# 4ment/physher

Hardware: NVIDIA B200
Metric: lnL+gradient throughput (site patterns x tree nodes per second) (higher is better)
Workload: dtype f64

## Files before the change

### physher_b200/csrc/phb_nuc4.cu

```cuda
#include "phb_ctx.cuh"

#include <math.h>
#include <stdlib.h>
#include <string.h>

#define NUC4_CHUNK PHBC_WALK_CHUNK
#define NUC4_NT 256
#ifndef NUC4_L2PF
#define NUC4_L2PF 1
#endif

struct Nuc4Params {
	int T, N, C, P, PB, root;
	int n_post, n_pre, nslots, ntiles;
	int include_root_freqs, compat;
	int nbatch, phases;
	long long mats_stride;
	int post_first_tips, pre_first_tips;
	double threshold;
	const uint8_t *tip_codes;
	const double *weights;
	const double *props;
	const phbc_post_op *post_ops;
	const phbc_pre_op *pre_ops;
	const double *post_mats;
	const double *pre_mats;
	double *lower;
	double *gacc;
	double *gstat;
	double *cta_lnl;
	double *pattern_lnl;
	double freqs[4];
	double fq[4];
	double wroot[4];
	double FQ[16];
	double FQ2[16];
	const double *rates;
	double *hacc;
};

__device__ __forceinline__ void matvec_smem(const double *__restrict__ M, const double (&x)[4], double (&y)[4]) {
	const double2 *M2 = reinterpret_cast<const double2 *>(M);
#pragma unroll
	for (int i = 0; i < 4; i++) {
		const double2 a = M2[2 * i], b = M2[2 * i + 1];
		y[i] = fma(a.x, x[0], fma(a.y, x[1], fma(b.x, x[2], b.y * x[3])));
	}
}

__device__ __forceinline__ void tip_message(const double *__restrict__ M, unsigned code, double (&y)[4]) {
	if (__all_sync(0xffffffffu, code < 4u)) {
#pragma unroll
		for (int i = 0; i < 4; i++) y[i] = M[4 * i + code];
	} else {
		double x[4];
#pragma unroll
		for (int j = 0; j < 4; j++) x[j] = (code < 4u ? code == (unsigned)j : ((code >> j) & 1u)) ? 1.0 : 0.0;
		matvec_smem(M, x, y);
		if (code == 4u) y[0] = y[1] = y[2] = y[3] = 1.0;
	}
}

#define NUC4_SLOT_BYTES (2 * NUC4_NT * 16)
#define NUC4_ROW_BYTES (NUC4_NT * 32)

__device__ __forceinline__ void cell_load(const unsigned char *cell, double (&x)[4]) {
	const double2 lo = *reinterpret_cast<const double2 *>(cell);
	const double2 hi = *reinterpret_cast<const double2 *>(cell + NUC4_NT * 16);
	x[0] = lo.x, x[1] = lo.y, x[2] = hi.x, x[3] = hi.y;
}
__device__ __forceinline__ void cell_store(unsigned char *cell, const double (&x)[4]) {
	*reinterpret_cast<double2 *>(cell) = make_double2(x[0], x[1]);
	*reinterpret_cast<double2 *>(cell + NUC4_NT * 16) = make_double2(x[2], x[3]);
}
__device__ __forceinline__ void row_load(const unsigned char *cell, double (&x)[4]) {
	const double2 lo = __ldcs(reinterpret_cast<const double2 *>(cell));
	const double2 hi = __ldcs(reinterpret_cast<const double2 *>(cell + NUC4_NT * 16));
	x[0] = lo.x, x[1] = lo.y, x[2] = hi.x, x[3] = hi.y;
}
__device__ __forceinline__ void row_store(unsigned char *cell, const double (&x)[4]) {
	__stcs(reinterpret_cast<double2 *>(cell), make_double2(x[0], x[1]));
	__stcs(reinterpret_cast<double2 *>(cell + NUC4_NT * 16), make_double2(x[2], x[3]));
}

struct Nuc4Stage {
	uint32_t desc_off, mat_off, code_off, bytes;
};
__host__ __device__ constexpr Nuc4Stage nuc4_stage_layout(int C, int PB) {
	return Nuc4Stage{64u, (uint32_t)(64 + NUC4_CHUNK * 48), (uint32_t)(64 + NUC4_CHUNK * 48 + NUC4_CHUNK * 3 * C * 128),
	                 (uint32_t)((64 + NUC4_CHUNK * 48 + NUC4_CHUNK * 3 * C * 128 + 2 * NUC4_CHUNK * PB + 127) & ~127)};
}

__device__ __forceinline__ double butterfly4(double v0, double v1, double v2, double v3, int lane) {
	const bool h16 = lane & 16, h8 = lane & 8;
	const double r01 = (h16 ? v1 : v0) + __shfl_xor_sync(0xffffffffu, h16 ? v0 : v1, 16);
	const double r23 = (h16 ? v3 : v2) + __shfl_xor_sync(0xffffffffu, h16 ? v2 : v3, 16);
	double r = (h8 ? r23 : r01) + __shfl_xor_sync(0xffffffffu, h8 ? r01 : r23, 8);
	r += __shfl_xor_sync(0xffffffffu, r, 4);
	r += __shfl_xor_sync(0xffffffffu, r, 2);
	r += __shfl_xor_sync(0xffffffffu, r, 1);
	return r;
}
__device__ __forceinline__ double butterfly2(double v0, double v1, int lane) {
	const bool h16 = lane & 16;
	double r = (h16 ? v1 : v0) + __shfl_xor_sync(0xffffffffu, h16 ? v0 : v1, 16);
	r += __shfl_xor_sync(0xffffffffu, r, 8);
	r += __shfl_xor_sync(0xffffffffu, r, 4);
	r += __shfl_xor_sync(0xffffffffu, r, 2);
	r += __shfl_xor_sync(0xffffffffu, r, 1);
	return r;
}

__device__ __forceinline__ void tip_vector(unsigned code, double (&x)[4]) {
#pragma unroll
	for (int j = 0; j < 4; j++) x[j] = (code < 4u ? code == (unsigned)j : (code == 4u || ((code >> j) & 1u))) ? 1.0 : 0.0;
}

template <int PPT>
__device__ __forceinline__ void gstat_add(const double (&t)[PPT][4], const double (&x)[PPT][4], double *row, int lane) {
	double v[16];
#pragma unroll
	for (int i = 0; i < 4; i++)
#pragma unroll
		for (int j = 0; j < 4; j++) {
			double a = t[0][i] * x[0][j];
#pragma unroll
			for (int u = 1; u < PPT; u++) a = fma(t[u][i], x[u][j], a);
			v[4 * i + j] = a;
		}
#pragma unroll
	for (int w = 8, off = 16; w >= 1; w >>= 1, off >>= 1) {
		const bool h = lane & off;
#pragma unroll
		for (int k = 0; k < w; k++) {
			const double keep = h ? v[w + k] : v[k], send = h ? v[k] : v[w + k];
			v[k] = keep + __shfl_xor_sync(0xffffffffu, send, off);
		}
	}
	v[0] += __shfl_xor_sync(0xffffffffu, v[0], 1);
	if (!(lane & 1)) red_add_f64(row + (lane >> 1), v[0]);
}

template <int PPT>
__device__ __forceinline__ void matvec_smem_n(const double *__restrict__ M, const double (&x)[PPT][4], double (&y)[PPT][4]) {
	const double2 *M2 = reinterpret_cast<const double2 *>(M);
#pragma unroll
	for (int i = 0; i < 4; i++) {
		const double2 a = M2[2 * i], b = M2[2 * i + 1];
#pragma unroll
		for (int u = 0; u < PPT; u++) y[u][i] = fma(a.x, x[u][0], fma(a.y, x[u][1], fma(b.x, x[u][2], b.y * x[u][3])));
	}
}

template <int C, bool SCALE, int GRAD, int PPT>
__global__ void __launch_bounds__(NUC4_NT / PPT, GRAD == 3 ? (PPT == 1 ? 1 : 2) : 3) k_nuc4_walk(const Nuc4Params prm) {
	extern __shared__ __align__(128) unsigned char smem_raw[];
	constexpr int PB = NUC4_NT / C;
	constexpr int NTHR = NUC4_NT / PPT;
	constexpr int PBT = PB / PPT;
	static_assert(PBT % 32 == 0 || PPT == 1, "a warp must not mix categories");
	static_assert(GRAD != 3 || !SCALE, "the Hessian walk is unscaled (rescaled evaluations take the resident-partials route)");
	constexpr bool RECOMP = GRAD == 1 && !SCALE;
	const int tid = threadIdx.x, lane = tid & 31, warp = tid >> 5;
	const int c = tid / PBT, pl0 = tid - c * PBT;
	const int cell0 = c * PB + pl0;
	constexpr Nuc4Stage lay = nuc4_stage_layout(C, PB);
	uint64_t *bars = reinterpret_cast<uint64_t *>(smem_raw);
	unsigned char *stage0 = smem_raw;
	unsigned char *slot_cell = stage0 + 2 * lay.bytes + cell0 * 16;
	double *xch = reinterpret_cast<double *>(stage0 + 2 * lay.bytes + (size_t)prm.nslots * NUC4_SLOT_BYTES);
	double *invLw = xch + (SCALE ? (GRAD == 2 ? 5 : 4) : (GRAD == 3 ? 2 : 1)) * C * PB;
	double *sfslot = invLw + PB;
	const uint32_t my_mat = lay.mat_off + c * 128;
	const uint32_t my_code = lay.code_off + pl0;

	if (tid == 0) {
		mbar_init(&bars[0], 1);
		mbar_init(&bars[1], 1);
		asm volatile("fence.mbarrier_init.release.cluster;" ::: "memory");
	}
	__syncthreads();

	uint32_t loads = 0;
	const double prop_c = (C == 1) ? 1.0 : prm.props[c];
	double cta_lnl = 0.0;
	unsigned char *row_cell = GRAD ? reinterpret_cast<unsigned char *>(prm.lower) + (size_t)blockIdx.x * prm.n_post * NUC4_ROW_BYTES + cell0 * 16 : nullptr;
	double *my_gacc = nullptr;
	double *my_gstat = GRAD == 2 ? prm.gstat + ((size_t)blockIdx.x * (NTHR / 32) + warp) * prm.N * 16 : nullptr;
	double *my_hacc = GRAD == 3 ? prm.hacc + ((size_t)blockIdx.x * (NTHR / 32) + warp) * prm.N : nullptr;
	const double rate_c = GRAD == 3 ? prm.rates[c] : 0.0;

	constexpr int PF_LPR = PPT * 2 * 4;
	const int pf_row = (lane / PF_LPR) & 1, pf_q = lane % PF_LPR;
	const bool pf_on = GRAD && lane < 2 * PF_LPR;
	const unsigned char *pf_base = GRAD ? row_cell - lane * 16 + ((pf_q >> 3) * PBT) * 16 + ((pf_q >> 2) & 1) * (NUC4_NT * 16) + (pf_q & 3) * 128 : nullptr;

	const long long nitems = (long long)prm.ntiles * prm.nbatch;
	const bool strided = prm.nbatch == 1;
	const int item0 = strided ? (int)blockIdx.x : (int)(blockIdx.x * nitems / gridDim.x);
	const int item1 = strided ? (int)nitems : (int)((blockIdx.x + 1) * nitems / gridDim.x);
	const int item_step = strided ? (int)gridDim.x : 1;
	const int b_first = strided ? 0 : item0 / prm.ntiles;
	int cur_b = -1;
	auto flush_lnl = [&](int b) {
		if (lane == 0) prm.cta_lnl[((size_t)blockIdx.x * prm.phases + (b - b_first)) * (NTHR / 32) + warp] = (c == 0) ? cta_lnl : 0.0;
	};

	for (int item = item0; item < item1; item += item_step) {
		const int bsmp = item / prm.ntiles, tile = item - bsmp * prm.ntiles;
		if (bsmp != cur_b) {
			if (cur_b >= 0) flush_lnl(cur_b);
			cur_b = bsmp;
			cta_lnl = 0.0;
			if (GRAD) my_gacc = prm.gacc + (((size_t)blockIdx.x * prm.phases + (bsmp - b_first)) * (NTHR / 32) + warp) * prm.N;
		}
		const uint8_t *tile_codes_post = prm.tip_codes + (size_t)tile * prm.T * PB;
		const uint8_t *tile_codes_pre = prm.tip_codes + ((size_t)prm.ntiles + tile) * prm.T * PB;

		double out[PPT][4];
		double sf_acc[PPT];
#pragma unroll
		for (int u = 0; u < PPT; u++) out[u][0] = out[u][1] = out[u][2] = out[u][3] = 1.0, sf_acc[u] = 0.0;
		{
			const int nchunks = (prm.n_post + NUC4_CHUNK - 1) / NUC4_CHUNK;
			auto issue = [&](int ch, uint32_t ld, int tips) {
				const int first = ch * NUC4_CHUNK;
				const int cnt = min(NUC4_CHUNK, prm.n_post - first);
				unsigned char *dst = stage0 + (ld & 1) * lay.bytes;
				const uint32_t dbytes = cnt * (uint32_t)sizeof(phbc_post_op), mbytes = cnt * 3 * C * 128;
				const uint32_t cbytes = (tips & 31) * PB;
				mbar_expect_tx(&bars[ld & 1], dbytes + mbytes + cbytes);
				bulk_g2s(dst + lay.desc_off, prm.post_ops + first, dbytes, &bars[ld & 1]);
				bulk_g2s(dst + lay.mat_off, prm.post_mats + (size_t)cur_b * prm.mats_stride + (size_t)first * 3 * C * 16, mbytes, &bars[ld & 1]);
				if (cbytes) bulk_g2s(dst + lay.code_off, tile_codes_post + (size_t)(tips >> 5) * PB, cbytes, &bars[ld & 1]);
			};
			if (tid == 0) issue(0, loads, prm.post_first_tips);
			for (int ch = 0; ch < nchunks; ch++) {
				mbar_wait(&bars[loads & 1], (loads >> 1) & 1);
				const unsigned char *st = stage0 + (loads & 1) * lay.bytes;
				const phbc_post_op *desc = reinterpret_cast<const phbc_post_op *>(st + lay.desc_off);
				if (tid == 0 && ch + 1 < nchunks) issue(ch + 1, loads + 1, desc[0].next_tips);
				const unsigned char *mats = st + my_mat;
				const uint8_t *cds = st + my_code;
				const int first = ch * NUC4_CHUNK;
				const int cnt = min(NUC4_CHUNK, prm.n_post - first);
#pragma unroll 1
				for (int j = 0; j < cnt; j++) {
					const int kind = (desc[j].a_kind & 0xff) + desc[j].b_kind;
					const bool keep_row = !(RECOMP && (desc[j].a_kind & PHBC_POST_NO_ROW));
					const int a_idx = desc[j].a_idx, b_idx = desc[j].b_idx, dst_slot = desc[j].dst_slot;
					const double *MN = reinterpret_cast<const double *>(mats + (j * 3 + 0) * C * 128);
					const double *MA = reinterpret_cast<const double *>(mats + (j * 3 + 1) * C * 128);
					const double *MB = reinterpret_cast<const double *>(mats + (j * 3 + 2) * C * 128);
					double ma[PPT][4], lw[PPT][4];
					double sf_in[PPT];
#pragma unroll
					for (int u = 0; u < PPT; u++) sf_in[u] = 0.0;
					if (kind == 0) {
#pragma unroll
						for (int u = 0; u < PPT; u++) {
							tip_message(MA, cds[a_idx * PB + u * PBT], ma[u]);
							tip_message(MB, cds[b_idx * PB + u * PBT], out[u]);
						}
					} else {
						if (SCALE) {
#pragma unroll
							for (int u = 0; u < PPT; u++) sf_in[u] = sf_acc[u];
						}
						if (kind == 1) {
#pragma unroll
							for (int u = 0; u < PPT; u++) tip_message(MA, cds[a_idx * PB + u * PBT], ma[u]);
						} else {
#pragma unroll
							for (int u = 0; u < PPT; u++) {
								cell_load(slot_cell + a_idx * NUC4_SLOT_BYTES + u * PBT * 16, ma[u]);
								if (SCALE) sf_in[u] += sfslot[a_idx * NUC4_NT + cell0 + u * PBT];
							}
						}
					}
#pragma unroll
					for (int u = 0; u < PPT; u++)
#pragma unroll
						for (int i = 0; i < 4; i++) lw[u][i] = ma[u][i] * out[u][i];
					if (SCALE) {
						double *mx = xch + ((first + j) & 1) * C * PB;
#pragma unroll
						for (int u = 0; u < PPT; u++) mx[cell0 + u * PBT] = fmax(fmax(lw[u][0], lw[u][1]), fmax(lw[u][2], lw[u][3]));
						__syncthreads();
#pragma unroll
						for (int u = 0; u < PPT; u++) {
							const int pl = pl0 + u * PBT;
							double m = mx[pl];
							for (int cc = 1; cc < C; cc++) m = fmax(m, mx[cc * PB + pl]);
							double sf = 0.0;
							if (m < prm.threshold) {
#pragma unroll
								for (int i = 0; i < 4; i++) lw[u][i] /= m;
								sf = log(m);
							}
							sf_acc[u] = sf + sf_in[u];
							if (dst_slot >= 0) sfslot[dst_slot * NUC4_NT + cell0 + u * PBT] = sf_acc[u];
						}
					}
					matvec_smem_n<PPT>(MN, lw, out);
#pragma unroll
					for (int u = 0; u < PPT; u++) {
						if (dst_slot >= 0) cell_store(slot_cell + dst_slot * NUC4_SLOT_BYTES + u * PBT * 16, out[u]);
						if (GRAD && keep_row) row_store(row_cell + (size_t)(unsigned)(first + j) * NUC4_ROW_BYTES + u * PBT * 16, out[u]);
					}
				}
				loads++;
				__syncthreads();
			}
		}

		{
#pragma unroll
			for (int u = 0; u < PPT; u++) {
				double site = prm.freqs[0] * out[u][0] + prm.freqs[1] * out[u][1] + prm.freqs[2] * out[u][2] + prm.freqs[3] * out[u][3];
				xch[cell0 + u * PBT] = site * prop_c;
			}
			__syncthreads();
			if (c == 0) {
				double v = 0.0;
#pragma unroll
				for (int u = 0; u < PPT; u++) {
					const int pl = pl0 + u * PBT;
					const int p = tile * PB + pl;
					const bool live = p < prm.P;
					double L = xch[pl];
					for (int cc = 1; cc < C; cc++) L += xch[cc * PB + pl];
					double plk = log(L);
					if (SCALE) plk += sf_acc[u];
					const double w = live ? prm.weights[p] : 0.0;
					if (live && prm.nbatch == 1) prm.pattern_lnl[p] = plk;
					invLw[pl] = w / L;
					if (GRAD == 3) invLw[PB + pl] = 1.0 / L;
					v += live ? plk * w : 0.0;
				}
				v = phb_warp_sum(v);
				if (lane == 0) cta_lnl += v;
			}
			__syncthreads();
		}

		if (GRAD) {
			double sgrad[PPT], wk[PPT], rinv[PPT];
#pragma unroll
			for (int u = 0; u < PPT; u++) {
				const int pl = pl0 + u * PBT;
				const int p = tile * PB + pl;
				sgrad[u] = invLw[pl];
				wk[u] = p < prm.P ? prm.weights[p] : 0.0;
				rinv[u] = GRAD == 3 ? invLw[PB + pl] : 0.0;
			}
			if (GRAD == 2) {
				double r[4];
#pragma unroll
				for (int i = 0; i < 4; i++) {
					r[i] = sgrad[0] * out[0][i];
#pragma unroll
					for (int u = 1; u < PPT; u++) r[i] = fma(sgrad[u], out[u][i], r[i]);
				}
				const double tot = butterfly4(r[0], r[1], r[2], r[3], lane);
				if ((lane & 7) == 0) red_add_f64(my_gstat + (size_t)prm.root * 16 + (((lane >> 4) & 1) | ((lane >> 2) & 2)), tot);
			}
			const int nchunks = (prm.n_pre + NUC4_CHUNK - 1) / NUC4_CHUNK;
			auto issue = [&](int ch, uint32_t ld, int tips) {
				const int first = ch * NUC4_CHUNK;
				const int cnt = min(NUC4_CHUNK, prm.n_pre - first);
				unsigned char *dst = stage0 + (ld & 1) * lay.bytes;
				const uint32_t dbytes = cnt * (uint32_t)sizeof(phbc_pre_op), mbytes = cnt * 3 * C * 128;
				const uint32_t cbytes = (tips & 31) * PB;
				mbar_expect_tx(&bars[ld & 1], dbytes + mbytes + cbytes);
				bulk_g2s(dst + lay.desc_off, prm.pre_ops + first, dbytes, &bars[ld & 1]);
				bulk_g2s(dst + lay.mat_off, prm.pre_mats + (size_t)cur_b * prm.mats_stride + (size_t)first * 3 * C * 16, mbytes, &bars[ld & 1]);
				if (cbytes) bulk_g2s(dst + lay.code_off, tile_codes_pre + (size_t)(tips >> 5) * PB, cbytes, &bars[ld & 1]);
			};
			auto fetch = [&](const phbc_pre_op *d, double (&A)[PPT][4], double (&B)[PPT][4]) {
				const int kind = d->kind;
				const bool b_row = kind != 0 && !(RECOMP && (d->flags & PHBC_PRE_B_RECOMPUTE));
#pragma unroll
				for (int u = 0; u < PPT; u++) {
					if (kind == 2) row_load(row_cell + (size_t)(unsigned)d->a_row * NUC4_ROW_BYTES + u * PBT * 16, A[u]);
					if (b_row) row_load(row_cell + (size_t)(unsigned)d->b_row * NUC4_ROW_BYTES + u * PBT * 16, B[u]);
				}
			};
			constexpr bool ALT = GRAD != 2;
			constexpr bool L2PF = NUC4_L2PF && GRAD != 2;
			auto pre_op = [&](const phbc_pre_op *desc, const unsigned char *mats, const uint8_t *cds, int j, int cnt, bool more_chunks,
			                  double (&xa)[PPT][4], double (&xb)[PPT][4], double (&na_)[PPT][4], double (&nb_)[PPT][4], double (&ureg)[PPT][4],
			                  double &va, double &vb, double &ha, double &hb) {
				const phbc_pre_op *d = desc + j;
				const int kind = d->kind;
				auto prefetch = [&]() {
					if (j + 1 < cnt) {
						fetch(d + 1, na_, nb_);
					} else if (more_chunks) {
						mbar_wait(&bars[(loads + 1) & 1], ((loads + 1) >> 1) & 1);
						fetch(reinterpret_cast<const phbc_pre_op *>(stage0 + ((loads + 1) & 1) * lay.bytes + lay.desc_off), na_, nb_);
					}
				};
				auto recompute_b = [&]() {
					const bool same = j + 1 < cnt;
					const unsigned char *nst = same ? nullptr : stage0 + ((loads + 1) & 1) * lay.bytes;
					const phbc_pre_op *dn = same ? d + 1 : reinterpret_cast<const phbc_pre_op *>(nst + lay.desc_off);
					const unsigned char *nm = same ? mats + (j + 1) * 3 * C * 128 : nst + my_mat;
					const uint8_t *nc = same ? cds : nst + my_code;
					const double *NP = reinterpret_cast<const double *>(nm);
					const double *NA = reinterpret_cast<const double *>(nm + C * 128);
					const double *NB = reinterpret_cast<const double *>(nm + 2 * C * 128);
					double lb[PPT][4];
#pragma unroll
					for (int u = 0; u < PPT; u++) {
						tip_message(NA, nc[dn->a_code * PB + u * PBT], na_[u]);
						tip_message(NB, nc[dn->b_code * PB + u * PBT], nb_[u]);
#pragma unroll
						for (int i = 0; i < 4; i++) lb[u][i] = na_[u][i] * nb_[u][i];
					}
					matvec_smem_n<PPT>(NP, lb, xb);
				};
				if (L2PF) {
					const int r = reinterpret_cast<const int *>(&d->pf_a_row)[pf_row];
					if (pf_on && r >= 0) asm volatile("prefetch.global.L2 [%0];" ::"l"(pf_base + (size_t)(unsigned)r * NUC4_ROW_BYTES));
				}
				const double *MP = reinterpret_cast<const double *>(mats + (j * 3 + 0) * C * 128);
				const double *MA = reinterpret_cast<const double *>(mats + (j * 3 + 1) * C * 128);
				const double *MB = reinterpret_cast<const double *>(mats + (j * 3 + 2) * C * 128);
				if (ALT) prefetch();
				if (RECOMP && (d->flags & PHBC_PRE_B_RECOMPUTE)) recompute_b();
				double W[PPT][4];
				if (d->u_kind == PHBC_W_ROOT) {
#pragma unroll
					for (int u = 0; u < PPT; u++)
#pragma unroll
						for (int i = 0; i < 4; i++) W[u][i] = prm.wroot[i];
				} else {
					if (d->u_kind == PHBC_W_SLOT) {
#pragma unroll
						for (int u = 0; u < PPT; u++) cell_load(slot_cell + d->u_slot * NUC4_SLOT_BYTES + u * PBT * 16, ureg[u]);
					}
					matvec_smem_n<PPT>(MP, ureg, W);
				}
				auto body = [&](double (&ma)[PPT][4], double (&mb)[PPT][4]) {
				double ua[PPT][4], ub[PPT][4];
#pragma unroll
				for (int u = 0; u < PPT; u++)
#pragma unroll
					for (int i = 0; i < 4; i++) ua[u][i] = W[u][i] * mb[u][i], ub[u][i] = W[u][i] * ma[u][i];
				double na[PPT], nb[PPT], da[PPT], db[PPT];
#pragma unroll
				for (int u = 0; u < PPT; u++) na[u] = nb[u] = da[u] = db[u] = 0.0;
#pragma unroll
				for (int i = 0; i < 4; i++) {
#pragma unroll
					for (int u = 0; u < PPT; u++) {
						const double qa = fma(prm.FQ[4 * i], ma[u][0], fma(prm.FQ[4 * i + 1], ma[u][1], fma(prm.FQ[4 * i + 2], ma[u][2], prm.FQ[4 * i + 3] * ma[u][3])));
						const double qb = fma(prm.FQ[4 * i], mb[u][0], fma(prm.FQ[4 * i + 1], mb[u][1], fma(prm.FQ[4 * i + 2], mb[u][2], prm.FQ[4 * i + 3] * mb[u][3])));
						na[u] = fma(ua[u][i], qa, na[u]);
						nb[u] = fma(ub[u][i], qb, nb[u]);
						if (SCALE) {
							da[u] = fma(prm.fq[i] * ua[u][i], ma[u][i], da[u]);
							db[u] = fma(prm.fq[i] * ub[u][i], mb[u][i], db[u]);
						}
					}
				}
				va = vb = 0.0;
				double coefa[PPT], coefb[PPT], coefp[PPT];
#pragma unroll
				for (int u = 0; u < PPT; u++) coefa[u] = coefb[u] = coefp[u] = sgrad[u];
				if (!SCALE) {
#pragma unroll
					for (int u = 0; u < PPT; u++) va = fma(na[u], sgrad[u], va), vb = fma(nb[u], sgrad[u], vb);
					if (GRAD == 3) {
						double lpa[PPT], lpb[PPT];
						if (C == 1) {
#pragma unroll
							for (int u = 0; u < PPT; u++) lpa[u] = rate_c * na[u] * rinv[u], lpb[u] = rate_c * nb[u] * rinv[u];
						} else {
							const double pr = prm.props[c] * rate_c;
							__syncthreads();
#pragma unroll
							for (int u = 0; u < PPT; u++) {
								const int ci = cell0 + u * PBT;
								xch[ci] = na[u] * pr;
								xch[C * PB + ci] = nb[u] * pr;
							}
							__syncthreads();
#pragma unroll
							for (int u = 0; u < PPT; u++) {
								const int pl = pl0 + u * PBT;
								double sa = 0.0, sb = 0.0;
								for (int cc = 0; cc < C; cc++) sa += xch[cc * PB + pl], sb += xch[C * PB + cc * PB + pl];
								lpa[u] = sa * rinv[u], lpb[u] = sb * rinv[u];
							}
						}
						ha = hb = 0.0;
#pragma unroll
						for (int u = 0; u < PPT; u++) {
							double sa = 0.0, sb = 0.0;
#pragma unroll
							for (int i = 0; i < 4; i++) {
								const double qa = fma(prm.FQ2[4 * i], ma[u][0], fma(prm.FQ2[4 * i + 1], ma[u][1], fma(prm.FQ2[4 * i + 2], ma[u][2], prm.FQ2[4 * i + 3] * ma[u][3])));
								const double qb = fma(prm.FQ2[4 * i], mb[u][0], fma(prm.FQ2[4 * i + 1], mb[u][1], fma(prm.FQ2[4 * i + 2], mb[u][2], prm.FQ2[4 * i + 3] * mb[u][3])));
								sa = fma(ua[u][i], qa, sa);
								sb = fma(ub[u][i], qb, sb);
// ... 9 lines not shown
					for (int u = 0; u < PPT; u++) {
						const int ci = cell0 + u * PBT;
						plane[0 * C * PB + ci] = fmax(fmax(ua[u][0], ua[u][1]), fmax(ua[u][2], ua[u][3]));
						plane[1 * C * PB + ci] = fmax(fmax(ub[u][0], ub[u][1]), fmax(ub[u][2], ub[u][3]));
						plane[2 * C * PB + ci] = da[u] * prop_c;
						plane[3 * C * PB + ci] = db[u] * prop_c;
						if (GRAD == 2) {
							double dp = 0.0;
#pragma unroll
							for (int i = 0; i < 4; i++) dp = fma(prm.fq[i] * W[u][i], ma[u][i] * mb[u][i], dp);
							plane[4 * C * PB + ci] = dp * prop_c;
						}
					}
					__syncthreads();
#pragma unroll
					for (int u = 0; u < PPT; u++) {
						const int pl = pl0 + u * PBT;
						double mxa = 0.0, mxb = 0.0, dta = 0.0, dtb = 0.0;
						for (int cc = 0; cc < C; cc++) {
							mxa = fmax(mxa, plane[0 * C * PB + cc * PB + pl]);
							mxb = fmax(mxb, plane[1 * C * PB + cc * PB + pl]);
							dta += plane[2 * C * PB + cc * PB + pl];
							dtb += plane[3 * C * PB + cc * PB + pl];
						}
						if (mxa < prm.threshold) {
#pragma unroll
							for (int i = 0; i < 4; i++) ua[u][i] /= mxa;
						}
						if (mxb < prm.threshold) {
#pragma unroll
							for (int i = 0; i < 4; i++) ub[u][i] /= mxb;
						}
						va += prm.compat ? na[u] / da[u] * wk[u] : na[u] / dta * wk[u];
						vb += prm.compat ? nb[u] / db[u] * wk[u] : nb[u] / dtb * wk[u];
						if (GRAD == 2) {
							double dtp = 0.0;
							for (int cc = 0; cc < C; cc++) dtp += plane[4 * C * PB + cc * PB + pl];
							coefa[u] = wk[u] / dta * (mxa < prm.threshold ? mxa : 1.0);
							coefb[u] = wk[u] / dtb * (mxb < prm.threshold ? mxb : 1.0);
							coefp[u] = wk[u] / dtp;
						}
					}
				}
				if (GRAD == 2 && d->u_kind != PHBC_W_ROOT) {
					double tp[PPT][4], xp[PPT][4];
#pragma unroll
					for (int u = 0; u < PPT; u++)
#pragma unroll
						for (int i = 0; i < 4; i++) tp[u][i] = coefp[u] * prm.fq[i] * ureg[u][i], xp[u][i] = ma[u][i] * mb[u][i];
					gstat_add<PPT>(tp, xp, my_gstat + (size_t)d->node * 16, lane);
				}
				if (GRAD == 2 && kind != 2) {
					double tt[PPT][4], xt[PPT][4];
#pragma unroll
					for (int u = 0; u < PPT; u++) {
						tip_vector(cds[d->a_code * PB + u * PBT], xt[u]);
#pragma unroll
						for (int i = 0; i < 4; i++) tt[u][i] = coefa[u] * prm.fq[i] * ua[u][i];
					}
					gstat_add<PPT>(tt, xt, my_gstat + (size_t)d->a_node * 16, lane);
					if (kind == 0) {
#pragma unroll
						for (int u = 0; u < PPT; u++) {
							tip_vector(cds[d->b_code * PB + u * PBT], xt[u]);
#pragma unroll
							for (int i = 0; i < 4; i++) tt[u][i] = coefb[u] * prm.fq[i] * ub[u][i];
						}
						gstat_add<PPT>(tt, xt, my_gstat + (size_t)d->b_node * 16, lane);
					}
				}
#pragma unroll
				for (int u = 0; u < PPT; u++) {
					if (kind == 2) cell_store(slot_cell + d->a_slot * NUC4_SLOT_BYTES + u * PBT * 16, ua[u]);
#pragma unroll
					for (int i = 0; i < 4; i++) ureg[u][i] = ub[u][i];
				}
				};
				if (ALT) {
#pragma unroll
					const bool tips_ready = RECOMP && (d->flags & PHBC_PRE_TIPS_READY);
					if (!tips_ready) {
#pragma unroll
						for (int u = 0; u < PPT; u++) {
							if (kind != 2) tip_message(MA, cds[d->a_code * PB + u * PBT], xa[u]);
							if (kind == 0) tip_message(MB, cds[d->b_code * PB + u * PBT], xb[u]);
						}
					}
					body(xa, xb);
				} else {
					double la[PPT][4], lb[PPT][4];
#pragma unroll
					for (int u = 0; u < PPT; u++) {
						if (kind == 2) {
#pragma unroll
							for (int i = 0; i < 4; i++) la[u][i] = xa[u][i];
						} else tip_message(MA, cds[d->a_code * PB + u * PBT], la[u]);
						if (kind == 0) tip_message(MB, cds[d->b_code * PB + u * PBT], lb[u]);
						else {
#pragma unroll
							for (int i = 0; i < 4; i++) lb[u][i] = xb[u][i];
						}
					}
					prefetch();
					body(la, lb);
				}
			};
			if (tid == 0) issue(0, loads, prm.pre_first_tips);
			mbar_wait(&bars[loads & 1], (loads >> 1) & 1);
			static_assert(NUC4_CHUNK % 2 == 0, "the two operand register sets alternate in pairs of ops");
			double xa[PPT][4], xb[PPT][4], ya[PPT][4], yb[PPT][4], ureg[PPT][4];
#pragma unroll
			for (int u = 0; u < PPT; u++)
#pragma unroll
				for (int i = 0; i < 4; i++) xa[u][i] = xb[u][i] = ya[u][i] = yb[u][i] = ureg[u][i] = 0.0;
			fetch(reinterpret_cast<const phbc_pre_op *>(stage0 + (loads & 1) * lay.bytes + lay.desc_off), xa, xb);
			for (int ch = 0; ch < nchunks; ch++) {
				const unsigned char *st = stage0 + (loads & 1) * lay.bytes;
				const phbc_pre_op *desc = reinterpret_cast<const phbc_pre_op *>(st + lay.desc_off);
				if (tid == 0 && ch + 1 < nchunks) issue(ch + 1, loads + 1, desc[0].next_tips);
				const unsigned char *mats = st + my_mat;
				const uint8_t *cds = st + my_code;
				const int first = ch * NUC4_CHUNK;
				const int cnt = min(NUC4_CHUNK, prm.n_pre - first);
				const bool more = ch + 1 < nchunks;
#pragma unroll 1
				for (int j = 0; j < cnt; j += 2) {
					double v0, v1, v2 = 0.0, v3 = 0.0;
					double h0 = 0.0, h1 = 0.0, h2 = 0.0, h3 = 0.0;
					if (ALT) pre_op(desc, mats, cds, j, cnt, more, xa, xb, ya, yb, ureg, v0, v1, h0, h1);
					else pre_op(desc, mats, cds, j, cnt, more, xa, xb, xa, xb, ureg, v0, v1, h0, h1);
					if (j + 1 < cnt) {
						if (ALT) pre_op(desc, mats, cds, j + 1, cnt, more, ya, yb, xa, xb, ureg, v2, v3, h2, h3);
						else pre_op(desc, mats, cds, j + 1, cnt, more, xa, xb, xa, xb, ureg, v2, v3, h2, h3);
						const double r = butterfly4(v0, v1, v2, v3, lane);
						if ((lane & 7) == 0) {
							const phbc_pre_op *d = desc + j + ((lane >> 3) & 1);
							red_add_f64(my_gacc + ((lane & 16) ? d->b_node : d->a_node), r);
						}
						if (GRAD == 3) {
							const double rh = butterfly4(h0, h1, h2, h3, lane);
							if ((lane & 7) == 0) {
								const phbc_pre_op *d = desc + j + ((lane >> 3) & 1);
								red_add_f64(my_hacc + ((lane & 16) ? d->b_node : d->a_node), rh);
							}
						}
					} else {
						const double r = butterfly2(v0, v1, lane);
						if ((lane & 15) == 0) red_add_f64(my_gacc + ((lane & 16) ? desc[j].b_node : desc[j].a_node), r);
						if (GRAD == 3) {
							const double rh = butterfly2(h0, h1, lane);
							if ((lane & 15) == 0) red_add_f64(my_hacc + ((lane & 16) ? desc[j].b_node : desc[j].a_node), rh);
						}
					}
				}
				loads++;
				__syncthreads();
			}
		}
	}
	if (cur_b >= 0) flush_lnl(cur_b);
}

__global__ void k_nuc4_matrices(int T, int C, int root, int n_post, int n_pre, const phbc_post_op *__restrict__ post_ops,
                                const phbc_pre_op *__restrict__ pre_ops, const double *__restrict__ evec,
                                const double *__restrict__ eval, const double *__restrict__ ivec, const double *__restrict__ bl,
                                const double *__restrict__ rates, double *__restrict__ post_mats, double *__restrict__ pre_mats, int N,
                                long long mats_stride) {
	const int e = blockIdx.x * blockDim.x + threadIdx.x;
	const int total = (3 * n_post + 3 * n_pre) * C;
	if (e >= total) return;
	bl += (size_t)blockIdx.y * N;
	post_mats += (size_t)blockIdx.y * mats_stride;
	pre_mats += (size_t)blockIdx.y * mats_stride;
	const int c = e % C;
	const int m = e / C;
	int node, which;
	double *dst;
	if (m < 3 * n_post) {
		const phbc_post_op op = post_ops[m / 3];
		which = m % 3;
		node = which == 0 ? op.node : (which == 1 ? op.a_node : op.b_node);
		dst = post_mats + (size_t)e * 16;
	} else {
		const int mm = m - 3 * n_post;
		const phbc_pre_op op = pre_ops[mm / 3];
		which = mm % 3;
		node = which == 0 ? op.node : (which == 1 ? op.a_node : op.b_node);
		dst = pre_mats + ((size_t)mm * C + c) * 16;
	}
	if (which != 0 && node >= T) return;
	if (node == root) {
		const double diag = m < 3 * n_post ? 1.0 : 0.0;
#pragma unroll
		for (int k = 0; k < 16; k++) dst[k] = (k % 5 == 0) ? diag : 0.0;
		return;
	}
	const double t = bl[node] * rates[c];
	double ex[4];
#pragma unroll
	for (int k = 0; k < 4; k++) ex[k] = exp(eval[k] * t);
#pragma unroll
	for (int i = 0; i < 4; i++)
#pragma unroll
		for (int j = 0; j < 4; j++) {
			double acc = 0.0;
#pragma unroll
			for (int k = 0; k < 4; k++) acc = __dadd_rn(acc, __dmul_rn(__dmul_rn(ivec[k * 4 + j], ex[k]), evec[i * 4 + k]));
			dst[i * 4 + j] = fabs(acc);
		}
}

__global__ void k_nuc4_encode_tips(int T, int P, int PB, int ntiles, int tip_kind, const uint8_t *__restrict__ states,
                                   const double *__restrict__ partials, const int *__restrict__ post_order,
                                   const int *__restrict__ pre_order, uint8_t *__restrict__ codes, int *__restrict__ bad) {
	const size_t per_walk = (size_t)ntiles * T * PB;
	const size_t i = (size_t)blockIdx.x * blockDim.x + threadIdx.x;
	if (i >= 2 * per_walk) return;
	const int walk = i >= per_walk;
	const size_t r = i - walk * per_walk;
	const int pl = (int)(r % PB);
	const int k = (int)((r / PB) % T);
	const int tile = (int)(r / ((size_t)PB * T));
	const int p = tile * PB + pl;
	const int tip = walk ? pre_order[k] : post_order[k];
	unsigned code = 4;
	if (p < P) {
		if (tip_kind == PHBC_TIP_STATES) {
			const unsigned s = states[(size_t)tip * P + p];
			code = s < 4 ? s : 4;
		} else {
			unsigned mask = 0;
			for (int j = 0; j < 4; j++) {
				const double v = partials[((size_t)tip * P + p) * 4 + j];
				if (v == 1.0) mask |= 1u << j;
				else if (v != 0.0) *bad = 1;
			}
			code = __popc(mask) == 1 ? (unsigned)(__ffs(mask) - 1) : (0x10u | mask);
		}
	}
	codes[i] = (uint8_t)code;
}

#define NUC4_FY 16
__global__ void __launch_bounds__(32 * NUC4_FY) k_nuc4_finalize(int N, int C, int nw , int grid, int phases, int ntiles, int nbatch, int root,
                                                                const double *__restrict__ cta_lnl, const double *__restrict__ gacc, int want_grad,
                                                                const double *__restrict__ props, const double *__restrict__ rates,
                                                                double *__restrict__ cat_grad, double *__restrict__ result,
                                                                const double *__restrict__ hacc, double *__restrict__ hess) {
	constexpr int warps = NUC4_NT / 32;
	__shared__ double red[NUC4_FY][warps][33];
	const int wpc = nw / C;
	const int tx = threadIdx.x, ty = threadIdx.y;
	const int b = blockIdx.y;
	const long long nitems = (long long)ntiles * nbatch;
	const long long lo = (long long)b * ntiles, hi = lo + ntiles;
	int c_lo = 0, c_hi = grid;
	if (nbatch > 1) {
		c_lo = (int)(lo * grid / nitems);
		c_hi = (int)((hi * grid + nitems - 1) / nitems) + 1;
		while (c_lo > 0 && (long long)c_lo * nitems / grid > lo) c_lo--;
		if (c_hi > grid) c_hi = grid;
	}
	result += (size_t)b * (1 + N);
	cat_grad += (size_t)b * N * C;
	auto phase_of = [&](int cta) -> int {
		if (nbatch == 1) return 0;
		const long long i0 = (long long)cta * nitems / grid, i1 = (long long)(cta + 1) * nitems / grid;
		if (i1 <= lo || i0 >= hi || i1 <= i0) return -1;
		return b - (int)(i0 / ntiles);
	};
	if (blockIdx.x == 0) {
		double s = 0.0;
		for (int cta = c_lo + ty; cta < c_hi; cta += NUC4_FY) {
			const int ph = phase_of(cta);
			if (ph >= 0 && tx < nw) s += cta_lnl[((size_t)cta * phases + ph) * nw + tx];
		}
		s = phb_warp_sum(s);
		if (tx == 0) red[ty][0][32] = s;
		__syncthreads();
		if (tx == 0 && ty == 0) {
			double tot = 0.0;
			for (int k = 0; k < NUC4_FY; k++) tot += red[k][0][32];
			result[0] = tot;
		}
		__syncthreads();
	}
	if (!want_grad) return;
	const int n = blockIdx.x * 32 + tx;
	for (int set = 0; set < (hacc ? 2 : 1); set++) {
		const double *rows = set ? hacc : gacc;
		double s8[warps];
#pragma unroll
		for (int w = 0; w < warps; w++) s8[w] = 0.0;
		if (n < N && n != root)
			for (int cta = c_lo + ty; cta < c_hi; cta += NUC4_FY) {
				const int ph = phase_of(cta);
				if (ph < 0) continue;
				const double *base = rows + ((size_t)cta * phases + ph) * nw * N + n;
#pragma unroll
				for (int w = 0; w < warps; w++)
					if (w < nw) s8[w] += base[(size_t)w * N];
			}
#pragma unroll
		for (int w = 0; w < warps; w++) red[ty][w][tx] = s8[w];
		__syncthreads();
		if (ty < nw) {
			double tot = 0.0;
			for (int k = 0; k < NUC4_FY; k++) tot += red[k][ty][tx];
			red[0][ty][tx] = tot;
		}
		__syncthreads();
		if (ty == 0 && n < N) {
			double g = 0.0;
			for (int c = 0; c < C; c++) {
				double tot = 0.0;
				for (int w = 0; w < wpc; w++) tot += red[0][c * wpc + w][tx];
				if (set == 0) cat_grad[(size_t)n * C + c] = tot;
				if (C == 1) g = tot;
				else g = c == 0 ? tot * props[0] * rates[0] : g + tot * props[c] * rates[c];
			}
			if (set == 0) result[1 + n] = g;
			else hess[n] = C == 1 ? g * rates[0] : g;
		}
// ... 158 lines not shown
	}
	if (o->want_gradient) {
		const size_t lower_bytes = (size_t)grid * ctx->n_post * NUC4_ROW_BYTES;
		if (lower_bytes > ctx->walk_lower_bytes) {
			PHBC_CHECK(cudaStreamSynchronize(ctx->stream));
			if (ctx->d_walk_lower) cudaFree(ctx->d_walk_lower);
			ctx->d_walk_lower = NULL;
			ctx->walk_lower_bytes = 0;
			PHBC_CHECK(cudaMalloc((void **)&ctx->d_walk_lower, lower_bytes));
			ctx->walk_lower_bytes = lower_bytes;
		}
		const size_t gacc_bytes = (size_t)grid * phases * warps * N * sizeof(double);
		if (gacc_bytes > ctx->walk_gacc_bytes) {
			PHBC_CHECK(cudaStreamSynchronize(ctx->stream));
			if (ctx->d_walk_gacc) cudaFree(ctx->d_walk_gacc);
			ctx->d_walk_gacc = NULL;
			ctx->walk_gacc_bytes = 0;
			PHBC_CHECK(cudaMalloc((void **)&ctx->d_walk_gacc, gacc_bytes));
			ctx->walk_gacc_bytes = gacc_bytes;
		}
		PHBC_CHECK(cudaMemsetAsync(ctx->d_walk_gacc, 0, gacc_bytes, ctx->stream));
	}
	if (want_stat) {
		const size_t gstat_bytes = (size_t)grid * warps * N * 16 * sizeof(double);
		if (gstat_bytes > ctx->walk_gstat_bytes) {
			PHBC_CHECK(cudaStreamSynchronize(ctx->stream));
			if (ctx->d_walk_gstat) cudaFree(ctx->d_walk_gstat);
			ctx->d_walk_gstat = NULL;
			ctx->walk_gstat_bytes = 0;
			PHBC_CHECK(cudaMalloc((void **)&ctx->d_walk_gstat, gstat_bytes));
			ctx->walk_gstat_bytes = gstat_bytes;
		}
		if (!ctx->d_nuc4_G) PHBC_CHECK(cudaMalloc((void **)&ctx->d_nuc4_G, (size_t)N * C * 16 * sizeof(double)));
		PHBC_CHECK(cudaMemsetAsync(ctx->d_walk_gstat, 0, gstat_bytes, ctx->stream));
	}
	if (want_hess) {
		const size_t hacc_bytes = (size_t)grid * warps * N * sizeof(double);
		if (hacc_bytes > ctx->walk_hacc_bytes) {
			PHBC_CHECK(cudaStreamSynchronize(ctx->stream));
			if (ctx->d_walk_hacc) cudaFree(ctx->d_walk_hacc);
			ctx->d_walk_hacc = NULL;
			ctx->walk_hacc_bytes = 0;
			PHBC_CHECK(cudaMalloc((void **)&ctx->d_walk_hacc, hacc_bytes));
			ctx->walk_hacc_bytes = hacc_bytes;
		}
		if (!ctx->d_nuc4_hess) PHBC_CHECK(cudaMalloc((void **)&ctx->d_nuc4_hess, (size_t)N * sizeof(double)));
		PHBC_CHECK(cudaMemsetAsync(ctx->d_walk_hacc, 0, hacc_bytes, ctx->stream));
	}
	if (!ctx->d_nuc4_cta_lnl || ctx->nuc4_grid < grid * phases) {
		PHBC_CHECK(cudaStreamSynchronize(ctx->stream));
		if (ctx->d_nuc4_cta_lnl) cudaFree(ctx->d_nuc4_cta_lnl);
		ctx->d_nuc4_cta_lnl = NULL;
		ctx->nuc4_grid = 0;
		PHBC_CHECK(cudaMalloc((void **)&ctx->d_nuc4_cta_lnl, (size_t)grid * phases * warps * sizeof(double)));
		ctx->nuc4_grid = grid * phases;
	}
	if (nbatch > ctx->cat_grad_cap) {
		PHBC_CHECK(cudaStreamSynchronize(ctx->stream));
		cudaFree(ctx->d_cat_grad);
		ctx->d_cat_grad = NULL;
		ctx->cat_grad_cap = 0;
		PHBC_CHECK(cudaMalloc((void **)&ctx->d_cat_grad, (size_t)nbatch * N * C * sizeof(double)));
		ctx->cat_grad_cap = nbatch;
	}
	double *post_mats = ctx->d_walk_mats;
	double *pre_mats = ctx->d_walk_mats + (size_t)3 * ctx->n_post * C * 16;
	{
		const int total = (3 * ctx->n_post + 3 * ctx->n_pre) * C;
		k_nuc4_matrices<<<dim3((total + 127) / 128, nbatch), 128, 0, ctx->stream>>>(T, C, ctx->root, ctx->n_post, ctx->n_pre, ctx->d_post_ops, ctx->d_pre_ops,
		                                                                          ctx->d_evec, ctx->d_eval, ctx->d_ivec,
		                                                                          ctx->d_bl + (size_t)o->batch_index * N, ctx->d_rates, post_mats, pre_mats,
		                                                                          N, mats_stride);
		ctx->launches++;
	}
	Nuc4Params prm;
	memset(&prm, 0, sizeof(prm));
	prm.T = T, prm.N = N, prm.C = C, prm.P = P, prm.PB = PB, prm.root = ctx->root;
	prm.n_post = ctx->n_post, prm.n_pre = ctx->n_pre, prm.nslots = nslots, prm.ntiles = ntiles;
	prm.include_root_freqs = o->include_root_freqs, prm.compat = o->compat_scaled_gradient;
	prm.nbatch = nbatch, prm.phases = phases, prm.mats_stride = mats_stride;
	prm.post_first_tips = ctx->post_first_tips, prm.pre_first_tips = ctx->pre_first_tips;
	prm.threshold = o->scaling_threshold;
	prm.tip_codes = ctx->d_nuc4_codes;
	prm.weights = ctx->d_weights;
	prm.props = ctx->d_props;
	prm.post_ops = ctx->d_post_ops;
	prm.pre_ops = ctx->d_pre_ops;
	prm.post_mats = post_mats;
	prm.pre_mats = pre_mats;
	prm.lower = ctx->d_walk_lower;
	prm.gacc = ctx->d_walk_gacc;
	prm.gstat = ctx->d_walk_gstat;
	prm.cta_lnl = ctx->d_nuc4_cta_lnl;
	prm.pattern_lnl = ctx->d_pattern_lnl;
	memcpy(prm.freqs, ctx->h_freqs, sizeof(prm.freqs));
	const bool irf = o->include_root_freqs && !want_hess;
	for (int i = 0; i < 4; i++) {
		prm.fq[i] = irf ? 1.0 : ctx->h_freqs[i];
		prm.wroot[i] = irf ? ctx->h_freqs[i] : 1.0;
		for (int j = 0; j < 4; j++) prm.FQ[4 * i + j] = prm.fq[i] * ctx->h_qmat[4 * i + j];
	}
	if (want_hess) {
		for (int i = 0; i < 4; i++)
			for (int j = 0; j < 4; j++) {
				double q2 = 0.0;
				for (int k = 0; k < 4; k++) q2 += ctx->h_qmat[4 * i + k] * ctx->h_qmat[4 * k + j];
				prm.FQ2[4 * i + j] = ctx->h_freqs[i] * q2;
			}
		prm.rates = ctx->d_rates;
		prm.hacc = ctx->d_walk_hacc;
	}
	int trc;
	if ((trc = phbc_time_begin(ctx))) return trc;
	kern<<<grid, nthr, smem, ctx->stream>>>(prm);
	ctx->launches++;
	if ((trc = phbc_time_end(ctx))) return trc;
	double *result = ctx->d_result + (size_t)o->batch_index * (1 + N);
	k_nuc4_finalize<<<dim3((N + 31) / 32, nbatch), dim3(32, NUC4_FY), 0, ctx->stream>>>(N, C, warps, grid, phases, ntiles, nbatch, ctx->root, ctx->d_nuc4_cta_lnl,
	                                                                         ctx->d_walk_gacc, o->want_gradient, ctx->d_props, ctx->d_rates,
	                                                                         ctx->d_cat_grad, result, want_hess ? ctx->d_walk_hacc : NULL,
	                                                                         want_hess ? ctx->d_nuc4_hess : NULL);
	ctx->launches++;
	if (want_stat) {
		k_nuc4_gstat_sum<<<(N * C * 16 + 63) / 64, dim3(64, NUC4_GY), 0, ctx->stream>>>(N, C, warps, grid, ctx->d_walk_gstat, ctx->d_nuc4_G);
		ctx->launches++;
		ctx->nuc4_G_valid = true;
	}
	PHBC_CHECK(cudaGetLastError());
	return 0;
}

static int nuc4_prepare_codes(phbc_ctx *ctx, int *usable) {
	const int C = ctx->C, T = ctx->T, P = ctx->P;
	const int PB = pattern_block(C);
	const int ntiles = (P + PB - 1) / PB;
	if (!ctx->d_nuc4_codes) {
		PHBC_CHECK(cudaMalloc((void **)&ctx->d_nuc4_codes, 2 * (size_t)ntiles * T * PB));
		PHBC_CHECK(cudaMalloc((void **)&ctx->d_nuc4_bad, sizeof(int)));
	}
	if (!ctx->nuc4_codes_valid) {
		const size_t n = 2 * (size_t)ntiles * T * PB;
		PHBC_CHECK(cudaMemsetAsync(ctx->d_nuc4_bad, 0, sizeof(int), ctx->stream));
		k_nuc4_encode_tips<<<(unsigned)((n + 255) / 256), 256, 0, ctx->stream>>>(T, P, PB, ntiles, ctx->tip_kind, ctx->d_tip_states, ctx->d_tip_partials,
		                                                                       ctx->d_post_tip_order, ctx->d_pre_tip_order, ctx->d_nuc4_codes,
		                                                                       ctx->d_nuc4_bad);
		ctx->launches++;
		int bad = 0;
		PHBC_CHECK(cudaMemcpyAsync(&bad, ctx->d_nuc4_bad, sizeof(int), cudaMemcpyDeviceToHost, ctx->stream));
		PHBC_CHECK(cudaStreamSynchronize(ctx->stream));
		ctx->nuc4_codes_bad = bad != 0;
		ctx->nuc4_codes_valid = true;
	}
	*usable = !ctx->nuc4_codes_bad;
	return 0;
}

int phbc_nuc4_matrix_gradient(phbc_ctx *ctx, const phbc_eval_opts *o, int nsets, const double *M_host, int skip_node, double *lnl, double *out_host) {
	phbc_eval_opts e = *o;
	e.want_gradient = 2;
	e.batch_count = 1;
	if (o->kernels == 1 || !phbc_nuc4_supported(ctx, &e)) return 1;
	if (o->scale) {
		if (o->include_root_freqs || o->compat_scaled_gradient) return 1;
		double worst = 0.0, big = 0.0;
		for (int i = 0; i < 4; i++)
			for (int j = 0; j < 4; j++) {
				const double a = ctx->h_freqs[i] * ctx->h_qmat[4 * i + j], b = ctx->h_freqs[j] * ctx->h_qmat[4 * j + i];
				worst = fmax(worst, fabs(a - b));
				big = fmax(big, fabs(a));
			}
		if (!(worst <= 1e-12 * big)) return 1;
	}
	PHBC_CHECK(cudaSetDevice(ctx->device));
	int usable = 0, rc;
	if ((rc = nuc4_prepare_codes(ctx, &usable))) return rc;
	if (!usable) return 1;
	if ((rc = phbc_nuc4_evaluate(ctx, &e))) return rc;
	const size_t N = ctx->N, C = ctx->C, set = N * C * 16;
	if ((rc = phbc_ensure_scratch(ctx, ((size_t)nsets * set + nsets) * sizeof(double)))) return rc;
	double *d_M = ctx->d_scratch, *d_out = ctx->d_scratch + (size_t)nsets * set;
	PHBC_CHECK(cudaMemcpyAsync(d_M, M_host, (size_t)nsets * set * sizeof(double), cudaMemcpyHostToDevice, ctx->stream));
	k_nuc4_gstat_contract<<<nsets, 256, 0, ctx->stream>>>((int)N, (int)C, ctx->root, skip_node, ctx->d_nuc4_G, d_M, ctx->d_props, d_out);
	ctx->launches++;
	PHBC_CHECK(cudaMemcpyAsync(out_host, d_out, (size_t)nsets * sizeof(double), cudaMemcpyDeviceToHost, ctx->stream));
	if (lnl) PHBC_CHECK(cudaMemcpyAsync(lnl, ctx->d_result + (size_t)e.batch_index * (1 + N), sizeof(double), cudaMemcpyDeviceToHost, ctx->stream));
	PHBC_CHECK(cudaStreamSynchronize(ctx->stream));
	PHBC_CHECK(cudaGetLastError());
	return 0;
}

int phbc_nuc4_hessian(phbc_ctx *ctx, const phbc_eval_opts *o, double *lnl, double *grad, double *hess) {
	phbc_eval_opts e = *o;
	e.want_gradient = 3;
	e.batch_count = 1;
	e.include_root_freqs = 0;
	e.compat_scaled_gradient = 0;
	if (o->kernels == 1 || o->scale || o->batch_count > 1 || !phbc_nuc4_supported(ctx, &e)) return 1;
	PHBC_CHECK(cudaSetDevice(ctx->device));
	int usable = 0, rc;
	if ((rc = nuc4_prepare_codes(ctx, &usable))) return rc;
	if (!usable) return 1;
	if ((rc = phbc_nuc4_evaluate(ctx, &e))) return rc;
	PHBC_CHECK(cudaMemcpyAsync(hess, ctx->d_nuc4_hess, (size_t)ctx->N * sizeof(double), cudaMemcpyDeviceToHost, ctx->stream));
	if ((rc = phbc_download_results(ctx, 1, lnl, grad))) return rc;
	return 0;
}

int phbc_nuc4_root_frequency_gradient(phbc_ctx *ctx, double *out_host) {
	if (!ctx->nuc4_G_valid) {
		snprintf(phbc_errbuf, sizeof(phbc_errbuf), "transition statistics are not resident");
		return -4;
	}
	PHBC_CHECK(cudaSetDevice(ctx->device));
	double g[8 * 16], props[8];
	const int C = ctx->C;
	PHBC_CHECK(cudaMemcpyAsync(g, ctx->d_nuc4_G + (size_t)ctx->root * C * 16, (size_t)C * 16 * sizeof(double), cudaMemcpyDeviceToHost, ctx->stream));
	PHBC_CHECK(cudaMemcpyAsync(props, ctx->d_props, (size_t)C * sizeof(double), cudaMemcpyDeviceToHost, ctx->stream));
	PHBC_CHECK(cudaStreamSynchronize(ctx->stream));
	for (int i = 0; i < 4; i++) {
		double s = 0.0;
		for (int c = 0; c < C; c++) s += (C == 1 ? 1.0 : props[c]) * g[c * 16 + i];
		out_host[i] = s;
	}
	return 0;
}

int phbc_nuc4_download_matrices(phbc_ctx *ctx, double *P, double *dP) {
	PHBC_CHECK(cudaSetDevice(ctx->device));
	if (!ctx->d_walk_mats) return -4;
	const int C = ctx->C, N = ctx->N, np = ctx->n_post;
	double *mats = (double *)malloc((size_t)3 * np * C * 16 * sizeof(double));
	phbc_post_op *ops = (phbc_post_op *)malloc((size_t)np * sizeof(phbc_post_op));
	double *Pl = P ? P : (double *)malloc((size_t)N * C * 16 * sizeof(double));
	if (!mats || !ops || !Pl) {
		free(mats), free(ops);
		if (!P) free(Pl);
		return -3;
	}
	cudaError_t e = cudaMemcpyAsync(mats, ctx->d_walk_mats, (size_t)3 * np * C * 16 * sizeof(double), cudaMemcpyDeviceToHost, ctx->stream);
	if (e == cudaSuccess) e = cudaMemcpyAsync(ops, ctx->d_post_ops, (size_t)np * sizeof(phbc_post_op), cudaMemcpyDeviceToHost, ctx->stream);
	if (e == cudaSuccess) e = cudaStreamSynchronize(ctx->stream);
	if (e == cudaSuccess) {
		memset(Pl, 0, (size_t)N * C * 16 * sizeof(double));
		for (int k = 0; k < np; k++) {
			const int node[3] = {ops[k].node, (ops[k].a_kind & 0xff) == PHBC_W_TIP ? ops[k].a_node : -1, ops[k].b_kind == PHBC_W_TIP ? ops[k].b_node : -1};
			for (int w = 0; w < 3; w++)
				if (node[w] >= 0) memcpy(Pl + (size_t)node[w] * C * 16, mats + ((size_t)3 * k + w) * C * 16, (size_t)C * 16 * sizeof(double));
		}
		if (dP)
			for (int nc = 0; nc < N * C; nc++)
				for (int i = 0; i < 4; i++)
					for (int j = 0; j < 4; j++) {
						double acc = 0.0;
						for (int k = 0; k < 4; k++) acc += ctx->h_qmat[4 * i + k] * Pl[(size_t)nc * 16 + 4 * k + j];
						dP[(size_t)nc * 16 + 4 * i + j] = acc;
					}
	}
	free(mats), free(ops);
	if (!P) free(Pl);
	PHBC_CHECK(e);
	return 0;
}
```

Baseline: 35.74 billion.

## Store tip transition matrices transposed and skip warp vote on ambiguity-free tiles

Tip-branch transition matrices are now written transposed, so a tip message for an unambiguous state becomes one contiguous column read as two double2 loads instead of four strided scalar loads. A per-tile 'plain' flag, computed during tip encoding, lets the kernel skip the __all_sync warp vote when a tile has no ambiguous codes. Pre-order descriptors are also loaded as 16-byte vectors into registers when PPT==2. The host-side matrix readback un-transposes to stay consistent. This adds one byte per tile of storage and assumes every other consumer of the tip matrices handles the new layout.

```diff
diff --git a/physher_b200/csrc/phb_nuc4.cu b/physher_b200/csrc/phb_nuc4.cu
--- a/physher_b200/csrc/phb_nuc4.cu
+++ b/physher_b200/csrc/phb_nuc4.cu
@@ -19,6 +19,7 @@
 	int post_first_tips, pre_first_tips;
 	double threshold;
 	const uint8_t *tip_codes;
+	const uint8_t *tile_plain;
 	const double *weights;
 	const double *props;
 	const phbc_post_op *post_ops;
@@ -39,24 +40,17 @@
 	double *hacc;
 };
 
-__device__ __forceinline__ void matvec_smem(const double *__restrict__ M, const double (&x)[4], double (&y)[4]) {
-	const double2 *M2 = reinterpret_cast<const double2 *>(M);
-#pragma unroll
-	for (int i = 0; i < 4; i++) {
-		const double2 a = M2[2 * i], b = M2[2 * i + 1];
-		y[i] = fma(a.x, x[0], fma(a.y, x[1], fma(b.x, x[2], b.y * x[3])));
-	}
-}
-
-__device__ __forceinline__ void tip_message(const double *__restrict__ M, unsigned code, double (&y)[4]) {
-	if (__all_sync(0xffffffffu, code < 4u)) {
-#pragma unroll
-		for (int i = 0; i < 4; i++) y[i] = M[4 * i + code];
+__device__ __forceinline__ void tip_message(const double *__restrict__ MT, unsigned code, bool plain, double (&y)[4]) {
+	if (plain || __all_sync(0xffffffffu, code < 4u)) {
+		const double2 *col = reinterpret_cast<const double2 *>(MT + 4 * code);
+		const double2 lo = col[0], hi = col[1];
+		y[0] = lo.x, y[1] = lo.y, y[2] = hi.x, y[3] = hi.y;
 	} else {
 		double x[4];
 #pragma unroll
 		for (int j = 0; j < 4; j++) x[j] = (code < 4u ? code == (unsigned)j : ((code >> j) & 1u)) ? 1.0 : 0.0;
-		matvec_smem(M, x, y);
+#pragma unroll
+		for (int i = 0; i < 4; i++) y[i] = fma(MT[i], x[0], fma(MT[4 + i], x[1], fma(MT[8 + i], x[2], MT[12 + i] * x[3])));
 		if (code == 4u) y[0] = y[1] = y[2] = y[3] = 1.0;
 	}
 }
@@ -216,6 +210,7 @@
 		}
 		const uint8_t *tile_codes_post = prm.tip_codes + (size_t)tile * prm.T * PB;
 		const uint8_t *tile_codes_pre = prm.tip_codes + ((size_t)prm.ntiles + tile) * prm.T * PB;
+		const bool plain = prm.tile_plain[tile];
 
 		double out[PPT][4];
 		double sf_acc[PPT];
@@ -259,8 +254,8 @@
 					if (kind == 0) {
 #pragma unroll
 						for (int u = 0; u < PPT; u++) {
-							tip_message(MA, cds[a_idx * PB + u * PBT], ma[u]);
-							tip_message(MB, cds[b_idx * PB + u * PBT], out[u]);
+							tip_message(MA, cds[a_idx * PB + u * PBT], plain, ma[u]);
+							tip_message(MB, cds[b_idx * PB + u * PBT], plain, out[u]);
 						}
 					} else {
 						if (SCALE) {
@@ -269,7 +264,7 @@
 						}
 						if (kind == 1) {
 #pragma unroll
-							for (int u = 0; u < PPT; u++) tip_message(MA, cds[a_idx * PB + u * PBT], ma[u]);
+							for (int u = 0; u < PPT; u++) tip_message(MA, cds[a_idx * PB + u * PBT], plain, ma[u]);
 						} else {
 #pragma unroll
 							for (int u = 0; u < PPT; u++) {
@@ -391,11 +386,18 @@
 			auto pre_op = [&](const phbc_pre_op *desc, const unsigned char *mats, const uint8_t *cds, int j, int cnt, bool more_chunks,
 			                  double (&xa)[PPT][4], double (&xb)[PPT][4], double (&na_)[PPT][4], double (&nb_)[PPT][4], double (&ureg)[PPT][4],
 			                  double &va, double &vb, double &ha, double &hb) {
-				const phbc_pre_op *d = desc + j;
+				const phbc_pre_op *dp = desc + j;
+				union {
+					int4 v[3];
+					phbc_pre_op o;
+				} dl;
+				if (PPT == 2) dl.v[0] = reinterpret_cast<const int4 *>(dp)[0], dl.v[1] = reinterpret_cast<const int4 *>(dp)[1], dl.v[2] = reinterpret_cast<const int4 *>(dp)[2];
+				static_assert(sizeof(phbc_pre_op) == 48 && NUC4_CHUNK * 48 % 16 == 0, "descriptors are read as 16-byte vectors");
+				const phbc_pre_op *d = PPT == 2 ? &dl.o : dp;
 				const int kind = d->kind;
 				auto prefetch = [&]() {
 					if (j + 1 < cnt) {
-						fetch(d + 1, na_, nb_);
+						fetch(dp + 1, na_, nb_);
 					} else if (more_chunks) {
 						mbar_wait(&bars[(loads + 1) & 1], ((loads + 1) >> 1) & 1);
 						fetch(reinterpret_cast<const phbc_pre_op *>(stage0 + ((loads + 1) & 1) * lay.bytes + lay.desc_off), na_, nb_);
@@ -404,7 +406,7 @@
 				auto recompute_b = [&]() {
 					const bool same = j + 1 < cnt;
 					const unsigned char *nst = same ? nullptr : stage0 + ((loads + 1) & 1) * lay.bytes;
-					const phbc_pre_op *dn = same ? d + 1 : reinterpret_cast<const phbc_pre_op *>(nst + lay.desc_off);
+					const phbc_pre_op *dn = same ? dp + 1 : reinterpret_cast<const phbc_pre_op *>(nst + lay.desc_off);
 					const unsigned char *nm = same ? mats + (j + 1) * 3 * C * 128 : nst + my_mat;
 					const uint8_t *nc = same ? cds : nst + my_code;
 					const double *NP = reinterpret_cast<const double *>(nm);
@@ -413,15 +415,15 @@
 					double lb[PPT][4];
 #pragma unroll
 					for (int u = 0; u < PPT; u++) {
-						tip_message(NA, nc[dn->a_code * PB + u * PBT], na_[u]);
-						tip_message(NB, nc[dn->b_code * PB + u * PBT], nb_[u]);
+						tip_message(NA, nc[dn->a_code * PB + u * PBT], plain, na_[u]);
+						tip_message(NB, nc[dn->b_code * PB + u * PBT], plain, nb_[u]);
 #pragma unroll
 						for (int i = 0; i < 4; i++) lb[u][i] = na_[u][i] * nb_[u][i];
 					}
 					matvec_smem_n<PPT>(NP, lb, xb);
 				};
 				if (L2PF) {
-					const int r = reinterpret_cast<const int *>(&d->pf_a_row)[pf_row];
+					const int r = pf_row ? d->pf_b_row : d->pf_a_row;
 					if (pf_on && r >= 0) asm volatile("prefetch.global.L2 [%0];" ::"l"(pf_base + (size_t)(unsigned)r * NUC4_ROW_BYTES));
 				}
 				const double *MP = reinterpret_cast<const double *>(mats + (j * 3 + 0) * C * 128);
@@ -597,8 +599,8 @@
 					if (!tips_ready) {
 #pragma unroll
 						for (int u = 0; u < PPT; u++) {
-							if (kind != 2) tip_message(MA, cds[d->a_code * PB + u * PBT], xa[u]);
-							if (kind == 0) tip_message(MB, cds[d->b_code * PB + u * PBT], xb[u]);
+							if (kind != 2) tip_message(MA, cds[d->a_code * PB + u * PBT], plain, xa[u]);
+							if (kind == 0) tip_message(MB, cds[d->b_code * PB + u * PBT], plain, xb[u]);
 						}
 					}
 					body(xa, xb);
@@ -609,8 +611,8 @@
 						if (kind == 2) {
 #pragma unroll
 							for (int i = 0; i < 4; i++) la[u][i] = xa[u][i];
-						} else tip_message(MA, cds[d->a_code * PB + u * PBT], la[u]);
-						if (kind == 0) tip_message(MB, cds[d->b_code * PB + u * PBT], lb[u]);
+						} else tip_message(MA, cds[d->a_code * PB + u * PBT], plain, la[u]);
+						if (kind == 0) tip_message(MB, cds[d->b_code * PB + u * PBT], plain, lb[u]);
 						else {
 #pragma unroll
 							for (int i = 0; i < 4; i++) lb[u][i] = xb[u][i];
@@ -721,13 +723,14 @@
 			double acc = 0.0;
 #pragma unroll
 			for (int k = 0; k < 4; k++) acc = __dadd_rn(acc, __dmul_rn(__dmul_rn(ivec[k * 4 + j], ex[k]), evec[i * 4 + k]));
-			dst[i * 4 + j] = fabs(acc);
+			dst[which ? j * 4 + i : i * 4 + j] = fabs(acc);
 		}
 }
 
 __global__ void k_nuc4_encode_tips(int T, int P, int PB, int ntiles, int tip_kind, const uint8_t *__restrict__ states,
                                    const double *__restrict__ partials, const int *__restrict__ post_order,
-                                   const int *__restrict__ pre_order, uint8_t *__restrict__ codes, int *__restrict__ bad) {
+                                   const int *__restrict__ pre_order, uint8_t *__restrict__ codes, uint8_t *__restrict__ plain,
+                                   int *__restrict__ bad) {
 	const size_t per_walk = (size_t)ntiles * T * PB;
 	const size_t i = (size_t)blockIdx.x * blockDim.x + threadIdx.x;
 	if (i >= 2 * per_walk) return;
@@ -754,6 +757,7 @@
 		}
 	}
 	codes[i] = (uint8_t)code;
+	if (code >= 4 && !walk) plain[tile] = 0;
 }
 
 #define NUC4_FY 16
@@ -1078,6 +1082,7 @@
 	prm.post_first_tips = ctx->post_first_tips, prm.pre_first_tips = ctx->pre_first_tips;
 	prm.threshold = o->scaling_threshold;
 	prm.tip_codes = ctx->d_nuc4_codes;
+	prm.tile_plain = ctx->d_nuc4_codes + 2 * (size_t)ntiles * T * PB;
 	prm.weights = ctx->d_weights;
 	prm.props = ctx->d_props;
 	prm.post_ops = ctx->d_post_ops;
@@ -1131,15 +1136,16 @@
 	const int PB = pattern_block(C);
 	const int ntiles = (P + PB - 1) / PB;
 	if (!ctx->d_nuc4_codes) {
-		PHBC_CHECK(cudaMalloc((void **)&ctx->d_nuc4_codes, 2 * (size_t)ntiles * T * PB));
+		PHBC_CHECK(cudaMalloc((void **)&ctx->d_nuc4_codes, 2 * (size_t)ntiles * T * PB + ntiles));
 		PHBC_CHECK(cudaMalloc((void **)&ctx->d_nuc4_bad, sizeof(int)));
 	}
 	if (!ctx->nuc4_codes_valid) {
 		const size_t n = 2 * (size_t)ntiles * T * PB;
 		PHBC_CHECK(cudaMemsetAsync(ctx->d_nuc4_bad, 0, sizeof(int), ctx->stream));
+		PHBC_CHECK(cudaMemsetAsync(ctx->d_nuc4_codes + n, 1, ntiles, ctx->stream));
 		k_nuc4_encode_tips<<<(unsigned)((n + 255) / 256), 256, 0, ctx->stream>>>(T, P, PB, ntiles, ctx->tip_kind, ctx->d_tip_states, ctx->d_tip_partials,
 		                                                                       ctx->d_post_tip_order, ctx->d_pre_tip_order, ctx->d_nuc4_codes,
-		                                                                       ctx->d_nuc4_bad);
+		                                                                       ctx->d_nuc4_codes + n, ctx->d_nuc4_bad);
 		ctx->launches++;
 		int bad = 0;
 		PHBC_CHECK(cudaMemcpyAsync(&bad, ctx->d_nuc4_bad, sizeof(int), cudaMemcpyDeviceToHost, ctx->stream));
@@ -1241,7 +1247,10 @@
 		for (int k = 0; k < np; k++) {
 			const int node[3] = {ops[k].node, (ops[k].a_kind & 0xff) == PHBC_W_TIP ? ops[k].a_node : -1, ops[k].b_kind == PHBC_W_TIP ? ops[k].b_node : -1};
 			for (int w = 0; w < 3; w++)
-				if (node[w] >= 0) memcpy(Pl + (size_t)node[w] * C * 16, mats + ((size_t)3 * k + w) * C * 16, (size_t)C * 16 * sizeof(double));
+				if (node[w] >= 0)
+					for (int c = 0; c < C; c++)
+						for (int e = 0; e < 16; e++)
+							Pl[((size_t)node[w] * C + c) * 16 + e] = mats[(((size_t)3 * k + w) * C + c) * 16 + (w ? (e % 4) * 4 + e / 4 : e)];
 		}
 		if (dP)
 			for (int nc = 0; nc < N * C; nc++)
```

Result: faster. 36.72 billion, median of 6 (+2.7%).
